# karpathy/minbpe

Measured on NVIDIA H100. Metric: train_loop_corpus_GBps, higher is better.
Workload: dtype int32

## Files before the change

### minbpe_b200/csrc/b200bpe.cu

```cuda
#include <algorithm>
#include <cstdio>
#include <cstdlib>
#include <cstring>
#include <new>
#include <string>
#include <vector>

#include "../../include/b200bpe.h"
#include "common.cuh"
#include "k_load.cuh"
#include "k_merge.cuh"
#include "k_merge_seg.cuh"
#include "k_seg.cuh"
#include "k_seg_filter.cuh"
#include "k_stats.cuh"
#include "k_encode.cuh"
#include "k_split.cuh"
#include "k_decode.cuh"
#include "k_xchg.cuh"
#include "k_encode2.cuh"
#include "k_special.cuh"
#include "k_weighted.cuh"
#include "k_dedup.cuh"

#define BPE_ABI_VERSION 4

struct EncState;
struct SpecSet;
struct GenEnc;
struct DdSession;
struct bpe_handle {
    int device = 0;
    EncState *enc = nullptr;
    bpe_handle *enc_scratch = nullptr;
    SpecSet *spec = nullptr;
    GenEnc *gen = nullptr;
    DdSession *dd = nullptr;
    int sms = 0;
    cudaStream_t stream = nullptr;
    cudaStream_t own_stream = nullptr;
    std::string err;

    u32 *buf[2] = {nullptr, nullptr};
    u64 cap_tokens = 0;
    bool loaded = false;
    bool bytes_only = false;
    bool weighted = false;
    u64 *wts = nullptr; u64 wts_cap = 0, n_entries = 0;
    u32 *wt_cnt = nullptr; u64 *wt_base = nullptr; u64 wt_seg_cap = 0;
    bool wt_fresh = false;

    Ctl *ctl = nullptr;
    Ctl *h_ctl = nullptr;

    Table table = {nullptr, nullptr, nullptr, 0};
    bool table_valid = false;
    u64 *desc = nullptr; u64 desc_cap = 0;
    Edge *edge[2] = {nullptr, nullptr}; u64 *seg_offs = nullptr; u64 seg_cap = 0;
    ull *delta = nullptr; u32 V = 0;
    u32 delta_cap = 0;
    u32 delta_vecs = 0;
    bool batching = false;
    u32 max_id = 255;
    ull *dense = nullptr;
    ull *dense2 = nullptr; u32 *d_cmp = nullptr;
    int hist_mode = 0;
    u32 *sig = nullptr, *cand = nullptr; u64 sig_cap = 0;
    bool filt_active = false;
    bool sig_valid = false;
    u32 *d_err = nullptr;
    int *log_pairs = nullptr; long long *log_counts = nullptr; int log_cap = 0;
    Best *partials = nullptr;
    TopList *top_partials = nullptr;
    unsigned char *d_cls = nullptr, *d_contr = nullptr;
    unsigned char *xchg = nullptr; u64 xchg_bytes = 0, xchg_stride = 0; u32 xchg_V = 0;
    XArgs xargs = {};
    bool xchg_attached = false;
    u32 *d_present = nullptr;
    unsigned char *split_slab = nullptr; u64 split_cap = 0;
    int argmax_grid = 0, merge_grid_same = 0, merge_grid_seg = 0, ff_grid = 0;

    int step_poll_every = 16;
    int opt_kernel_timing = 0, opt_rescan = 0, opt_batch = 256, opt_table_log2 = 0;
    int opt_memo_log2 = 0;
    u32 opt_vocab_cap = 0;
    int opt_seg_filter = 0;
    int opt_hist_kernel = 2;
    int opt_dedup_log2 = 0;
    u64 dd_stats[8] = {};
    int opt_split_pattern = 0;

    bpe_timing tm = {};
    std::vector<cudaEvent_t> ev_pool;
    int ev_used = 0;
};

static thread_local std::string g_create_err;
static void xchg_release(bpe_handle *h);
static void enc2_free(bpe_handle *h);
static void spec_free(bpe_handle *h);
static void gen_free(bpe_handle *h);
static void dd_free(bpe_handle *h);
static u64 g_split_piece_override = 0;

static int fail(bpe_handle *h, int code, const std::string &msg) {
    if (h) h->err = msg; else g_create_err = msg;
    return code;
}

#define CU(call)                                                                                   \
    do {                                                                                           \
        cudaError_t e_ = (call);                                                                   \
        if (e_ != cudaSuccess)                                                                     \
            return fail(h, BPE_ERR_CUDA, std::string(#call) + ": " + cudaGetErrorString(e_));      \
    } while (0)

static inline int grid_for(u64 work_items, int threads, int max_blocks) {
    u64 b = (work_items + threads - 1) / threads;
    if (b < 1) b = 1;
    if (b > (u64)max_blocks) b = max_blocks;
    return (int)b;
}

extern "C" int bpe_abi_version(void) { return BPE_ABI_VERSION; }

extern "C" const char *bpe_last_error(const bpe_handle *h) { return h ? h->err.c_str() : g_create_err.c_str(); }

static int free_table(bpe_handle *h, Table &t) {
    if (t.keys) cudaFree(t.keys);
    if (t.counts) cudaFree(t.counts);
    if (t.first) cudaFree(t.first);
    t = {nullptr, nullptr, nullptr, 0};
    (void)h;
    return BPE_OK;
}

static int alloc_table(bpe_handle *h, Table &t, u64 cap, bool with_first) {
    t = {nullptr, nullptr, nullptr, cap - 1};
    CU(cudaMalloc(&t.keys, cap * 8));
    CU(cudaMalloc(&t.counts, cap * 8));
    if (with_first) CU(cudaMalloc(&t.first, cap * 8));
    CU(cudaMemsetAsync(t.keys, 0xff, cap * 8, h->stream));
    CU(cudaMemsetAsync(t.counts, 0, cap * 8, h->stream));
    if (with_first) CU(cudaMemsetAsync(t.first, 0xff, cap * 8, h->stream));
    return BPE_OK;
}

static u64 next_pow2(u64 x) { u64 p = 1; while (p < x) p <<= 1; return p; }

extern "C" int bpe_create(int device, bpe_handle **out) {
    bpe_handle *h = nullptr;
    if (!out) return fail(nullptr, BPE_ERR_ARG, "bpe_create: out is NULL");
    *out = nullptr;
    int ndev = 0;
    cudaError_t e = cudaGetDeviceCount(&ndev);
    if (e != cudaSuccess || ndev == 0)
        return fail(nullptr, BPE_ERR_CUDA, std::string("bpe_create: no CUDA device (") + cudaGetErrorString(e) +
                                               "); libb200bpe has no CPU fallback");
    if (device < 0 || device >= ndev) return fail(nullptr, BPE_ERR_ARG, "bpe_create: device index out of range");
    cudaDeviceProp prop;
    e = cudaGetDeviceProperties(&prop, device);
    if (e != cudaSuccess) return fail(nullptr, BPE_ERR_CUDA, cudaGetErrorString(e));
    if (prop.major != 9 || prop.minor != 0)
        return fail(nullptr, BPE_ERR_CUDA, std::string("bpe_create: device '") + prop.name + "' is sm_" +
                                               std::to_string(prop.major) + std::to_string(prop.minor) +
                                               "; this library contains sm_90a code only");
    h = new (std::nothrow) bpe_handle();
    if (!h) return fail(nullptr, BPE_ERR_INTERNAL, "out of host memory");
    h->device = device;
    h->sms = prop.multiProcessorCount;
    auto bail = [&](const char *what, cudaError_t ce) {
        std::string m = std::string(what) + ": " + cudaGetErrorString(ce);
        delete h;
        return fail(nullptr, BPE_ERR_CUDA, m);
    };
    if ((e = cudaSetDevice(device)) != cudaSuccess) return bail("cudaSetDevice", e);
    if ((e = cudaStreamCreateWithFlags(&h->own_stream, cudaStreamNonBlocking)) != cudaSuccess) return bail("cudaStreamCreate", e);
    h->stream = h->own_stream;
    if ((e = cudaMalloc(&h->ctl, sizeof(Ctl))) != cudaSuccess) return bail("cudaMalloc ctl", e);
    if ((e = cudaMallocHost(&h->h_ctl, sizeof(Ctl))) != cudaSuccess) return bail("cudaMallocHost", e);
    if ((e = cudaMalloc(&h->dense, 65536 * 8)) != cudaSuccess) return bail("cudaMalloc dense", e);
    if ((e = cudaMalloc(&h->d_err, 8)) != cudaSuccess) return bail("cudaMalloc err", e);
    int occ_same = 1;
    cudaOccupancyMaxActiveBlocksPerMultiprocessor(&occ_same, k_merge<true>, MG_THREADS, 0);
    if (occ_same < 1) occ_same = 1;
    h->merge_grid_same = h->sms * occ_same;
    int occ_fast = 0;
    if ((e = cudaFuncSetAttribute(k_merge_seg<false>, cudaFuncAttributeMaxDynamicSharedMemorySize, MS_SMEM_BYTES)) != cudaSuccess)
        return bail("cudaFuncSetAttribute(k_merge_seg)", e);
    cudaOccupancyMaxActiveBlocksPerMultiprocessor(&occ_fast, k_merge_seg<false>, MS_THREADS, MS_SMEM_BYTES);
    if (occ_fast < 1) return bail("k_merge_seg does not fit on an SM", cudaErrorLaunchOutOfResources);
    h->merge_grid_seg = h->sms * occ_fast;
    h->argmax_grid = h->sms * 2;
    h->ff_grid = h->sms * 4;
    if ((e = cudaMalloc(&h->partials, sizeof(Best) * h->argmax_grid)) != cudaSuccess) return bail("cudaMalloc partials", e);
    if ((e = cudaMalloc(&h->top_partials, sizeof(TopList) * h->argmax_grid)) != cudaSuccess) return bail("cudaMalloc top_partials", e);
    memset(h->h_ctl, 0, sizeof(Ctl));
    h->h_ctl->epoch = 1;
    h->h_ctl->found_pos = POS_NONE;
    if ((e = cudaMemcpy(h->ctl, h->h_ctl, sizeof(Ctl), cudaMemcpyHostToDevice)) != cudaSuccess) return bail("cudaMemcpy ctl", e);
    *out = h;
    return BPE_OK;
}

extern "C" int bpe_destroy(bpe_handle *h) {
    if (!h) return BPE_OK;
    cudaSetDevice(h->device);
    cudaStreamSynchronize(h->stream);
    for (int i = 0; i < 2; ++i) if (h->buf[i]) cudaFree(h->buf[i]);
    for (cudaEvent_t e : h->ev_pool) cudaEventDestroy(e);
    free_table(h, h->table);
    if (h->desc) cudaFree(h->desc);
    for (int i = 0; i < 2; ++i) if (h->edge[i]) cudaFree(h->edge[i]);
    if (h->seg_offs) cudaFree(h->seg_offs);
    if (h->sig) cudaFree(h->sig);
    if (h->cand) cudaFree(h->cand);
    if (h->delta) cudaFree(h->delta);
    if (h->dense) cudaFree(h->dense);
    if (h->dense2) cudaFree(h->dense2);
    if (h->d_cmp) cudaFree(h->d_cmp);
    if (h->d_err) cudaFree(h->d_err);
    if (h->log_pairs) cudaFree(h->log_pairs);
    if (h->log_counts) cudaFree(h->log_counts);
    if (h->partials) cudaFree(h->partials);
    if (h->top_partials) cudaFree(h->top_partials);
    if (h->d_cls) cudaFree(h->d_cls);
    if (h->d_contr) cudaFree(h->d_contr);
    if (h->d_present) cudaFree(h->d_present);
    if (h->wts) cudaFree(h->wts);
    if (h->wt_cnt) cudaFree(h->wt_cnt);
    if (h->wt_base) cudaFree(h->wt_base);
    xchg_release(h);
    enc2_free(h);
    spec_free(h);
    gen_free(h);
    dd_free(h);
    if (h->enc_scratch) bpe_destroy(h->enc_scratch);
    if (h->split_slab) cudaFree(h->split_slab);
    if (h->ctl) cudaFree(h->ctl);
    if (h->h_ctl) cudaFreeHost(h->h_ctl);
    if (h->own_stream) cudaStreamDestroy(h->own_stream);
    delete h;
    return BPE_OK;
}

extern "C" int bpe_set_option(bpe_handle *h, int opt, int64_t value) {
    if (!h) return BPE_ERR_ARG;
    switch (opt) {
        case BPE_OPT_KERNEL_TIMING: h->opt_kernel_timing = value != 0; break;
        case BPE_OPT_RESCAN: h->opt_rescan = value != 0; break;
        case BPE_OPT_BATCH: h->opt_batch = (int)std::max<int64_t>(1, std::min<int64_t>(value, 4096)); break;
        case BPE_OPT_TABLE_LOG2:
            if (value != 0 && (value < 10 || value > 30)) return fail(h, BPE_ERR_ARG, "table log2 must be 0 or in [10,30]");
            h->opt_table_log2 = (int)value; break;
        case BPE_OPT_VOCAB_CAP:
            if (value < 0 || value >= 0x3fffffff) return fail(h, BPE_ERR_ARG, "vocabulary capacity out of range");
            h->opt_vocab_cap = (u32)value; break;
        case BPE_OPT_ENC_MEMO_LOG2:
            if (value != 0 && (value < 6 || value > 28)) return fail(h, BPE_ERR_ARG, "memo log2 must be 0 or in [6,28]");
            h->opt_memo_log2 = (int)value;
            cudaSetDevice(h->device); cudaStreamSynchronize(h->stream);
            enc2_free(h);
            break;
        case BPE_OPT_SEG_FILTER:
            if (value < 0 || value > 2) return fail(h, BPE_ERR_ARG, "segment filter must be 0 (off), 1 (when sparse) or 2 (always)");
            h->opt_seg_filter = (int)value; h->filt_active = false; h->sig_valid = false;
            break;
        case BPE_OPT_HIST_KERNEL:
            if (value < 0 || value > 2) return fail(h, BPE_ERR_ARG, "hist kernel must be 0 (auto), 1 (packed) or 2 (hashed)");
            h->opt_hist_kernel = (int)value;
            if (value == 0) h->hist_mode = 0;
            break;
        case BPE_OPT_SPLIT_PATTERN:
            if (value != 0 && value != 1) return fail(h, BPE_ERR_ARG, "split pattern must be 0 (GPT-4) or 1 (GPT-2)");
            h->opt_split_pattern = (int)value; break;
        case BPE_OPT_DEDUP_LOG2:
            if (value != 0 && (value < 4 || value > 30)) return fail(h, BPE_ERR_ARG, "dedup log2 must be 0 or in [4,30]");
            h->opt_dedup_log2 = (int)value; break;
        case BPE_OPT_SPLIT_PIECE:
            if (value != 0 && value < 4096) return fail(h, BPE_ERR_ARG, "split piece must be 0 (default) or >= 4096 bytes");
            g_split_piece_override = (u64)value; break;
        default: return fail(h, BPE_ERR_ARG, "unknown option");
    }
    return BPE_OK;
}

extern "C" int bpe_get_timing(bpe_handle *h, bpe_timing *out) {
    if (!h || !out) return BPE_ERR_ARG;
    *out = h->tm;
    return BPE_OK;
}

static int ensure_stream_capacity(bpe_handle *h, u64 n) {
    const u64 need = ((n + MG_TILE - 1) / MG_TILE + 1) * MG_TILE;
    if (need > h->cap_tokens) {
        if (h->split_slab) { cudaFree(h->split_slab); h->split_slab = nullptr; h->split_cap = 0; }
        for (int i = 0; i < 2; ++i) { if (h->buf[i]) cudaFree(h->buf[i]); h->buf[i] = nullptr; }
        h->cap_tokens = 0;
        for (int i = 0; i < 2; ++i) CU(cudaMalloc(&h->buf[i], need * 4));
        h->cap_tokens = need;
    }
    const u64 tiles = need / MG_TILE + 1;
    if (tiles > h->desc_cap) {
        if (h->desc) cudaFree(h->desc);
        h->desc = nullptr; h->desc_cap = 0;
        CU(cudaMalloc(&h->desc, tiles * 8));
        CU(cudaMemsetAsync(h->desc, 0, tiles * 8, h->stream));
        h->desc_cap = tiles;
    }
    const u64 segs = need / SEG_TOKENS + 1;
    if (segs > h->seg_cap) {
        for (int i = 0; i < 2; ++i) { if (h->edge[i]) cudaFree(h->edge[i]); h->edge[i] = nullptr; }
        if (h->seg_offs) cudaFree(h->seg_offs);
        h->seg_offs = nullptr; h->seg_cap = 0;
        for (int i = 0; i < 2; ++i) CU(cudaMalloc(&h->edge[i], segs * sizeof(Edge)));
        CU(cudaMalloc(&h->seg_offs, segs * 8));
        h->seg_cap = segs;
    }
    return BPE_OK;
}

static int build_edges(bpe_handle *h, u64 n) {
    const u64 nseg = (n + SEG_TOKENS - 1) / SEG_TOKENS;
    k_build_edges<<<grid_for(nseg, 256, h->sms * 4), 256, 0, h->stream>>>(h->buf[0], h->buf[1], h->ctl, h->edge[0], 0);
    CU(cudaGetLastError());
    return BPE_OK;
}

static void enqueue_pack(bpe_handle *h, int force) {
    k_scan_counts<<<1, 1024, 0, h->stream>>>(h->ctl, h->edge[0], h->edge[1], h->seg_offs, force);
    k_gather<<<h->sms * 8, 256, 0, h->stream>>>(h->ctl, h->buf[0], h->buf[1], h->edge[0], h->edge[1], h->seg_offs, nullptr, force, 1);
    h->tm.kernel_launches += 2;
}
static void enqueue_edges_after_contig(bpe_handle *h) {
    k_build_edges<<<h->sms * 4, 256, 0, h->stream>>>(h->buf[0], h->buf[1], h->ctl, h->edge[0], 1);
    h->tm.kernel_launches += 1;
}

static void enqueue_wt_bases(bpe_handle *h, int force) {
    k_wt_marks<<<h->sms * 8, 256, 0, h->stream>>>(h->buf[0], h->buf[1], h->ctl, h->edge[0], h->edge[1], h->wt_cnt, force);
    k_wt_scan<<<1, 1024, 0, h->stream>>>(h->ctl, h->wt_cnt, h->wt_base, force);
    h->tm.kernel_launches += 2;
}

static int push_ctl(bpe_handle *h) {
    CU(cudaMemcpyAsync(h->ctl, h->h_ctl, sizeof(Ctl), cudaMemcpyHostToDevice, h->stream));
    return BPE_OK;
}
static int pull_ctl(bpe_handle *h) {
    CU(cudaMemcpyAsync(h->h_ctl, h->ctl, sizeof(Ctl), cudaMemcpyDeviceToHost, h->stream));
    CU(cudaStreamSynchronize(h->stream));
    return BPE_OK;
}

static int reset_ctl_for_stream(bpe_handle *h, u64 n) {
    int rc = pull_ctl(h);
    if (rc) return rc;
    const u32 epoch = h->h_ctl->epoch ? h->h_ctl->epoch : 1;
    memset(h->h_ctl, 0, sizeof(Ctl));
    h->h_ctl->epoch = epoch;
    h->h_ctl->n = n;
    h->h_ctl->found_pos = POS_NONE;
    h->h_ctl->first_idx = 256;
    return push_ctl(h);
}

static int check_offsets(bpe_handle *h, const uint64_t *offs, uint64_t k, uint64_t n) {
    if (!offs || k == 0) return BPE_OK;
    if (offs[0] != 0) return fail(h, BPE_ERR_ARG, "chunk_offsets[0] must be 0");
    for (u64 i = 1; i < k; ++i)
        if (offs[i] <= offs[i - 1] || offs[i] >= n) return fail(h, BPE_ERR_ARG, "chunk_offsets must be strictly increasing and < n");
    return BPE_OK;
}

static int mark_chunks(bpe_handle *h, u32 *dst, const uint64_t *offs, uint64_t k, uint64_t n) {
    u64 zero = 0;
    if (!offs || k == 0) { offs = &zero; k = n ? 1 : 0; }
    if (k == 0) return BPE_OK;
    const u64 piece = 1ull << 24;
    u64 *d_offs = nullptr;
    CU(cudaMalloc(&d_offs, std::min(piece, k) * 8));
    for (u64 s = 0; s < k; s += piece) {
        const u64 m = std::min(piece, k - s);
        cudaError_t e = cudaMemcpyAsync(d_offs, offs + s, m * 8, cudaMemcpyHostToDevice, h->stream);
        if (e == cudaSuccess) {
            k_set_flags<<<grid_for(m, 256, h->sms * 8), 256, 0, h->stream>>>(dst, d_offs, m, n);
            e = cudaStreamSynchronize(h->stream);
        }
        if (e != cudaSuccess) { cudaFree(d_offs); return fail(h, BPE_ERR_CUDA, std::string("mark_chunks: ") + cudaGetErrorString(e)); }
        h->tm.h2d_bytes += m * 8;
    }
    cudaFree(d_offs);
    return BPE_OK;
}

static int load_bytes_into(bpe_handle *h, u32 *dst, const uint8_t *bytes, uint64_t n, const unsigned char *d_perm) {
    const u64 piece = 1ull << 28;
    unsigned char *d_bytes = nullptr;
    if (n == 0) return BPE_OK;
    CU(cudaMalloc(&d_bytes, std::min(piece, n)));
    for (u64 s = 0; s < n; s += piece) {
        const u64 m = std::min(piece, n - s);
        cudaError_t e = cudaMemcpyAsync(d_bytes, bytes + s, m, cudaMemcpyHostToDevice, h->stream);
        if (e == cudaSuccess) {
            k_widen_bytes<<<grid_for(m / 16 + 1, 256, h->sms * 8), 256, 0, h->stream>>>(d_bytes, dst + s, m, d_perm);
            e = cudaStreamSynchronize(h->stream);
        }
        if (e != cudaSuccess) { cudaFree(d_bytes); return fail(h, BPE_ERR_CUDA, std::string("load_bytes: ") + cudaGetErrorString(e)); }
        h->tm.h2d_bytes += m;
    }
    cudaFree(d_bytes);
    return BPE_OK;
}

extern "C" int bpe_load_stream(bpe_handle *h, const uint8_t *bytes, uint64_t n, const uint64_t *chunk_offsets,
                               uint64_t n_chunks) {
    if (!h) return BPE_ERR_ARG;
    if (!bytes && n) return fail(h, BPE_ERR_ARG, "bytes is NULL");
    if (n >= (1ull << 36)) return fail(h, BPE_ERR_ARG, "stream too long (limit 2^36 tokens)");
    CU(cudaSetDevice(h->device));
    int rc = check_offsets(h, chunk_offsets, n_chunks, n);
    if (rc) return rc;
    h->tm.h2d_bytes = 0;
    h->loaded = false; h->table_valid = false; h->weighted = false;
    if ((rc = ensure_stream_capacity(h, n))) return rc;
    if ((rc = load_bytes_into(h, h->buf[0], bytes, n, nullptr))) return rc;
    if ((rc = mark_chunks(h, h->buf[0], chunk_offsets, n_chunks, n))) return rc;
    if ((rc = reset_ctl_for_stream(h, n))) return rc;
    if ((rc = build_edges(h, n))) return rc;
    h->loaded = true; h->bytes_only = true; h->max_id = 255;
    return BPE_OK;
}

extern "C" int bpe_load_ids(bpe_handle *h, const int32_t *ids, uint64_t n, const uint64_t *chunk_offsets,
                            uint64_t n_chunks) {
    if (!h) return BPE_ERR_ARG;
    if (!ids && n) return fail(h, BPE_ERR_ARG, "ids is NULL");
    if (n >= (1ull << 36)) return fail(h, BPE_ERR_ARG, "stream too long (limit 2^36 tokens)");
    CU(cudaSetDevice(h->device));
    int rc = check_offsets(h, chunk_offsets, n_chunks, n);
    if (rc) return rc;
    h->tm.h2d_bytes = 0;
    h->loaded = false; h->table_valid = false; h->weighted = false;
    if ((rc = ensure_stream_capacity(h, n))) return rc;
    h->max_id = 0;
    if (n) {
        CU(cudaMemcpyAsync(h->buf[1], ids, n * 4, cudaMemcpyHostToDevice, h->stream));
        CU(cudaMemsetAsync(h->d_err, 0, 8, h->stream));
        k_copy_ids<<<grid_for(n, 256, h->sms * 8), 256, 0, h->stream>>>((const int *)h->buf[1], h->buf[0], n, h->d_err);
        u32 bad[2] = {0, 0};
        CU(cudaMemcpyAsync(bad, h->d_err, 8, cudaMemcpyDeviceToHost, h->stream));
        CU(cudaStreamSynchronize(h->stream));
        if (bad[0]) return fail(h, BPE_ERR_ARG, "ids must be in [0, 2^31-1)");
        h->max_id = bad[1];
        h->tm.h2d_bytes += n * 4;
    }
    if ((rc = mark_chunks(h, h->buf[0], chunk_offsets, n_chunks, n))) return rc;
    if ((rc = reset_ctl_for_stream(h, n))) return rc;
    if ((rc = build_edges(h, n))) return rc;
    h->loaded = true; h->bytes_only = false;
    return BPE_OK;
}

extern "C" int bpe_stream_len(bpe_handle *h, uint64_t *n) {
    if (!h || !n) return BPE_ERR_ARG;
    if (!h->loaded) return fail(h, BPE_ERR_STATE, "no stream loaded");
    CU(cudaSetDevice(h->device));
    int rc = pull_ctl(h);
    if (rc) return rc;
    *n = h->h_ctl->n;
    return BPE_OK;
}

extern "C" int bpe_read_stream(bpe_handle *h, int32_t *out, uint64_t cap, uint64_t *n) {
    if (!h || !n) return BPE_ERR_ARG;
    if (!h->loaded) return fail(h, BPE_ERR_STATE, "no stream loaded");
    CU(cudaSetDevice(h->device));
    int rc = pull_ctl(h);
    if (rc) return rc;
    const u64 len = h->h_ctl->n;
    *n = len;
    if (cap < len) return fail(h, BPE_ERR_CAPACITY, "output buffer too small");
    if (len == 0) return BPE_OK;
    if (!out) return fail(h, BPE_ERR_ARG, "out is NULL");
    const u32 cur = h->h_ctl->cur;
    k_scan_counts<<<1, 1024, 0, h->stream>>>(h->ctl, h->edge[0], h->edge[1], h->seg_offs, 1);
    k_gather<<<h->sms * 8, 256, 0, h->stream>>>(h->ctl, h->buf[0], h->buf[1], h->edge[0], h->edge[1], h->seg_offs,
                                                 h->buf[cur ^ 1], 1, 0);
    k_strip_flags<<<grid_for(len, 256, h->sms * 8), 256, 0, h->stream>>>(h->buf[cur ^ 1], (int *)h->buf[cur ^ 1], len);
    CU(cudaMemcpyAsync(out, h->buf[cur ^ 1], len * 4, cudaMemcpyDeviceToHost, h->stream));
    CU(cudaStreamSynchronize(h->stream));
// ... 530 lines not shown
```

### minbpe_b200/csrc/k_merge_seg.cuh

```cuda
#pragma once
#include "common.cuh"
#include "k_merge.cuh"
#include "k_seg.cuh"

#ifndef MS_WARPS
#define MS_WARPS 8
#endif
#define MS_THREADS (MS_WARPS * 32)
#ifndef MS_STAGES
#define MS_STAGES 2
#endif
#ifndef MS_MINBLOCKS
#define MS_MINBLOCKS 4
#endif
#ifndef MS_DCACHE_LOG2
#define MS_DCACHE_LOG2 9
#endif
#ifndef MS_BATCH
#define MS_BATCH 8
#endif
#define MS_PAD 4
#define MS_SW (SEG_TOKENS + 8)
#define MS_META 16
#define MS_BE (MS_BATCH + 2)
#define MS_DCACHE (1 << MS_DCACHE_LOG2)
#define MS_WARP_WORDS (MS_STAGES * MS_SW + MS_STAGES * MS_META + MS_BE * 8)
#define MS_SMEM_BYTES (MS_WARPS * MS_WARP_WORDS * 4 + MS_WARPS * MS_STAGES * 8 + MS_DCACHE * 8 + 16 + BATCH_MAX * 8)
#define MS_INVALID 0xffffffffu
static_assert(SEG_TOKENS == 512, "k_merge_seg: a lane owns 4 rows x 4 tokens of a 512-token segment");
static_assert((MS_SW * 4) % 16 == 0 && (MS_WARP_WORDS * 4) % 16 == 0, "bulk-copy destinations must stay 16-byte aligned");

__device__ __noinline__ void delta_cache_add(u32 *s_dkey, u32 *s_dcnt, ull *delta, u32 idx) {
    u32 slot = (idx * 2654435761u) >> (32 - MS_DCACHE_LOG2);
#pragma unroll 1
    for (int probe = 0; probe < 4; ++probe) {
        u32 k = reinterpret_cast<volatile u32 *>(s_dkey)[slot];
        if (k == 0xffffffffu) {
            const u32 old = atomicCAS(&s_dkey[slot], 0xffffffffu, idx);
            k = (old == 0xffffffffu) ? idx : old;
        }
        if (k == idx) { atomicAdd(&s_dcnt[slot], 1u); return; }
        slot = (slot + 1) & (MS_DCACHE - 1);
    }
    atomicAdd(&delta[idx], 1ull);
}

__device__ __noinline__ void delta_one(u32 at, u32 a, u32 b, u32 V, u32 *s_dkey, u32 *s_dcnt, ull *delta) {
    const u32 t0 = lds32(at), tm1 = lds32o<-4>(at), tm2 = lds32o<-8>(at), tp2 = lds32o<8>(at), tp3 = lds32o<12>(at);
    const bool m_m2 = (((tm2 ^ a) & TOK_MASK) == 0) && tm1 == b;
    const bool m_p2 = (((tp2 ^ a) & TOK_MASK) == 0) && tp3 == b;
    if (tm1 != TOK_SENTINEL && !(t0 & TOK_FLAG) && !m_m2) delta_cache_add(s_dkey, s_dcnt, delta, tm1 & TOK_MASK);
    if (!(tp2 & TOK_FLAG))
        delta_cache_add(s_dkey, s_dcnt, delta, m_p2 ? 2u * V : V + tp2);
}

__device__ __forceinline__ u32 batch_member(u32 tok, u32 nk, u32 mem_a) {
    u32 j = 0;
#pragma unroll 1
    for (; j < nk; ++j) if (lds32(mem_a + 8 * j) == (tok & TOK_MASK)) break;
    return j;
}
__device__ __forceinline__ u32 batch_start(u32 t, u32 nx, u32 nk, u32 mem_a) {
    const u32 j = batch_member(t, nk, mem_a);
    return (j < nk && lds32(mem_a + 8 * j + 4) == nx) ? j : nk;
}

__device__ __noinline__ void delta_batch(u32 at, u32 nk, u32 mem_a, u32 z, u32 V, u32 *s_dkey, u32 *s_dcnt, ull *delta) {
    const u32 t0 = lds32(at), tm1 = lds32o<-4>(at), tm2 = lds32o<-8>(at), tp2 = lds32o<8>(at), tp3 = lds32o<12>(at);
    const u32 j = batch_member(t0, nk, mem_a);
    const u32 ml = batch_start(tm2, tm1, nk, mem_a);
    const u32 mr = batch_start(tp2, tp3, nk, mem_a);
    const u32 base = j * (2u * V + 1u);
    if (tm1 != TOK_SENTINEL && !(t0 & TOK_FLAG) && ml != j)
        delta_cache_add(s_dkey, s_dcnt, delta, base + (ml < j ? z + ml : tm1 & TOK_MASK));
    if (!(tp2 & TOK_FLAG))
        delta_cache_add(s_dkey, s_dcnt, delta, base + (mr == j ? 2u * V : V + (mr < j ? z + mr : tp2)));
}

struct SegArgs {
    Ctl *ctl;
    u32 *buf0, *buf1;
    Edge *e0, *e1;
    ull *delta;
    u32 V;
    int force;
    int batched;
    const unsigned char *xbase;
    u64 xstride;
};

template <int R, bool BATCH>
__device__ __forceinline__ void mark_row(u32 la, u32 lane, u32 count, u32 a, u32 b, u32 z, u32 nk, u32 mem_a, u32 (&t)[4],
                                         u32 &mn, u32 &keep, u32 &dirty) {
    const uint4 q = lds128o<R * 512>(la);
    const u32 nx = lds32o<R * 512 + 16>(la), pv = lds32o<R * 512 - 4>(la);
    t[0] = q.x; t[1] = q.y; t[2] = q.z; t[3] = q.w;
    u32 m = 0, pm = 0;
#pragma unroll 1
    for (u32 j = 0; j < (BATCH ? nk : 1u); ++j) {
        if (BATCH) { a = lds32(mem_a + 8 * j); b = lds32(mem_a + 8 * j + 4); }
        m |= (((t[0] ^ a) & TOK_MASK) == 0 && t[1] == b) ? 1u : 0u;
        m |= (((t[1] ^ a) & TOK_MASK) == 0 && t[2] == b) ? 2u : 0u;
        m |= (((t[2] ^ a) & TOK_MASK) == 0 && t[3] == b) ? 4u : 0u;
        m |= (((t[3] ^ a) & TOK_MASK) == 0 && nx == b) ? 8u : 0u;
        pm |= (((pv ^ a) & TOK_MASK) == 0 && t[0] == b) ? 1u : 0u;
    }
    const u32 d = ((m << 1) | pm) & 0xfu;
    u32 valid = 0xfu;
    if (R * 128u + 128u > count) {
        const int rem = (int)count - (int)(R * 128 + lane * 4);
        valid = rem >= 4 ? 0xfu : (rem <= 0 ? 0u : ((1u << rem) - 1u));
    }
    mn = m & valid;
    keep = ~d & valid;
    dirty |= (mn | (keep ^ valid)) ? (1u << R) : 0u;
    if (mn) {
        auto zof = [&](u32 x) { return (BATCH ? z + batch_member(x, nk, mem_a) : z) | (x & TOK_FLAG); };
        if (mn & 1u) t[0] = zof(t[0]);
        if (mn & 2u) t[1] = zof(t[1]);
        if (mn & 4u) t[2] = zof(t[2]);
        if (mn & 8u) t[3] = zof(t[3]);
    }
}

__device__ __forceinline__ void scatter_row(u32 s_a, u32 lane, u32 off, u32 row_kept, u32 lane_excl, u32 kp, const u32 (&t)[4]) {
    if (row_kept == 128u) {
        const u32 p = s_a + ((off + 4u * lane) << 2);
        if ((off & 3u) == 0) sts128(p, t[0], t[1], t[2], t[3]);
        else { sts32(p, t[0]); sts32o<4>(p, t[1]); sts32o<8>(p, t[2]); sts32o<12>(p, t[3]); }
    } else {
        u32 p = s_a + ((off + lane_excl) << 2);
        if (kp & 1u) sts32(p, t[0]);
        p += (kp << 2) & 4u;
        if (kp & 2u) sts32(p, t[1]);
        p += (kp << 1) & 4u;
        if (kp & 4u) sts32(p, t[2]);
        p += kp & 4u;
        if (kp & 8u) sts32(p, t[3]);
    }
}

template <bool LIST>
__global__ void __launch_bounds__(MS_THREADS, MS_MINBLOCKS) k_merge_seg(SegArgs A) {
    Ctl *ctl = A.ctl;
    if (!A.force && (ctl->done || ctl->overflow || ctl->iter >= ctl->max_iter)) return;
    if (ctl->a == ctl->b) return;

    extern __shared__ __align__(128) unsigned char smem_raw[];
    u32 *s_warp = reinterpret_cast<u32 *>(smem_raw);
    u64 *s_bar = reinterpret_cast<u64 *>(s_warp + MS_WARPS * MS_WARP_WORDS);
    u32 *s_dkey = reinterpret_cast<u32 *>(s_bar + MS_WARPS * MS_STAGES);
    u32 *s_dcnt = s_dkey + MS_DCACHE;
    ull *s_drops = reinterpret_cast<ull *>(s_dcnt + MS_DCACHE);
    u32 *s_mem = reinterpret_cast<u32 *>(s_drops + 1);

    const u32 FULL = 0xffffffffu;
    const u32 tid = threadIdx.x, lane = tid & 31, warp = tid >> 5;
    const u64 n = ctl->n;
    u32 *__restrict__ w = ctl->cur ? A.buf1 : A.buf0;
    const Edge *__restrict__ e_cur = ctl->edge_cur ? A.e1 : A.e0;
    Edge *__restrict__ e_next = ctl->edge_cur ? A.e0 : A.e1;
    const u32 a = (u32)ctl->a, b = (u32)ctl->b, z = (u32)ctl->z;
    const u32 nseg = ctl->nseg;
    const u32 nk = (!LIST && A.batched) ? ctl->nk : 1u;
    const u32 mem_a = smem_addr(s_mem);
    ull *const delta = A.xbase ? x_local_delta(A.xbase, A.xstride) : A.delta;
    const u32 *__restrict__ cand = LIST ? reinterpret_cast<const u32 *>(ctl->cand_ptr) : nullptr;
    const u32 n_cand = LIST ? ctl->n_cand : 0u;

    const u32 ws_a = smem_addr(s_warp + warp * MS_WARP_WORDS);
    const u32 wmeta_a = ws_a + MS_STAGES * MS_SW * 4;
    const u32 wbe_a = wmeta_a + MS_STAGES * MS_META * 4;
    const u32 wbar_a = smem_addr(s_bar + warp * MS_STAGES);

    if (lane == 0) {
        for (int s = 0; s < MS_STAGES; ++s) mbar_init(s_bar + warp * MS_STAGES + s, 1);
        fence_mbar_init();
    }
    for (u32 i = tid; i < MS_DCACHE; i += MS_THREADS) { s_dkey[i] = 0xffffffffu; s_dcnt[i] = 0; }
    if (tid == 0) *s_drops = 0;
    if (tid < nk) { s_mem[2 * tid] = tid ? (u32)ctl->bat_a[tid] : a; s_mem[2 * tid + 1] = tid ? (u32)ctl->bat_b[tid] : b; }
    __syncthreads();

    u32 batch_seg = 0, batch_pos = MS_BATCH;
    u32 list_next = blockIdx.x * MS_WARPS + warp;
    const u32 meta_src = 4u * (lane == 0 ? 4u : lane == 1 ? 3u : lane < 5 ? 14u + lane : lane < 8 ? 0u : lane < 16 ? lane : 0u);
    bool exhausted = false;
    auto issue = [&](u32 stage) {
        const u32 meta_a = wmeta_a + stage * (MS_META * 4);
        for (;;) {
            if (exhausted) {
                if (lane == 0) sts32o<20>(meta_a, MS_INVALID);
                __syncwarp();
                return;
            }
            if (batch_pos == MS_BATCH) {
                u32 tk = 0;
                if (LIST) {
                    tk = list_next; list_next += gridDim.x * MS_WARPS;
                    if (tk >= n_cand) { exhausted = true; continue; }
                    batch_seg = cand[tk] - (MS_BATCH - 1); batch_pos = MS_BATCH - 1;
                } else {
                    if (lane == 0) tk = atomicAdd(&ctl->merge_ticket, 1u);
                    tk = __shfl_sync(FULL, tk, 0);
                    if ((u64)tk * MS_BATCH >= nseg) { exhausted = true; continue; }
                    batch_seg = tk * MS_BATCH; batch_pos = 0;
                }
                if (LIST ? (lane >= MS_BATCH - 1 && lane < MS_BE) : (lane < MS_BE)) {
                    const long long idx = (LIST ? (long long)(int)batch_seg : (long long)batch_seg) - 1 + lane;
                    uint4 q0, q1;
                    if (idx >= 0 && idx < (long long)nseg) {
                        const uint4 *p = reinterpret_cast<const uint4 *>(&e_cur[idx]);
                        q0 = p[0]; q1 = p[1];
                    } else {
                        q0 = make_uint4(TOK_SENTINEL, TOK_SENTINEL, TOK_SENTINEL, TOK_SENTINEL);
                        q1 = make_uint4(TOK_SENTINEL, 3u, 0u, 0u);
                    }
                    sts128(wbe_a + lane * 32, q0.x, q0.y, q0.z, q0.w);
                    sts128(wbe_a + lane * 32 + 16, q1.x, q1.y, q1.z, q1.w);
                }
                __syncwarp();
            }
            const u32 k = batch_pos++;
            const u32 seg = batch_seg + k;
            if (seg >= nseg) { exhausted = true; continue; }
            const u32 rec_a = wbe_a + k * 32;
            const u32 cnt = lds32o<32 + 20>(rec_a);
            if (cnt == 0) {
                if (lane < 8) reinterpret_cast<u32 *>(&e_next[seg])[lane] = (lane < 5) ? TOK_SENTINEL : 0u;
                continue;
            }
            const u32 cm1 = lds32o<20>(rec_a), cp1 = lds32o<64 + 20>(rec_a);
            const u32 st_a = ws_a + stage * (MS_SW * 4);
            u32 mv = lds32(rec_a + meta_src);
            if (lane == 5) mv = seg;
            if (lane == 6) mv = cnt;
            if (lane < 16) sts32(meta_a + lane * 4, mv);
            if (lane < 2) sts32(st_a + (MS_PAD - 1 - lane) * 4, mv);
            if (!(cm1 >= 2 && cp1 >= 3)) {
                __syncwarp();
                if (lane == 0) {
                    u32 N[3], P[2];
                    seg_neighbours(e_cur, seg, nseg, N, P);
                    sts32o<0>(meta_a, P[0]); sts32o<4>(meta_a, P[1]); sts32o<8>(meta_a, N[0]); sts32o<12>(meta_a, N[1]); sts32o<16>(meta_a, N[2]);
                    sts32o<(MS_PAD - 1) * 4>(st_a, P[0]); sts32o<(MS_PAD - 2) * 4>(st_a, P[1]);
                }
            }
            __syncwarp();
            if (lane == 0) {
                const u32 bytes = ((cnt + 3u) & ~3u) * 4u;
                fence_proxy_async_smem();
                mbar_arrive_expect_tx_a(wbar_a + stage * 8, bytes);
                bulk_g2s_a(st_a + MS_PAD * 4, w + (u64)seg * SEG_TOKENS, bytes, wbar_a + stage * 8);
            }
            __syncwarp();
            return;
        }
    };

    for (u32 s = 0; s + 1 < MS_STAGES; ++s) issue(s);
    u32 drops = 0;
    for (u32 j = 0;; ++j) {
        const u32 stage = j % MS_STAGES;
        issue((j + MS_STAGES - 1) % MS_STAGES);
        const u32 meta_a = wmeta_a + stage * (MS_META * 4);
        const u32 seg = lds32o<20>(meta_a);
        if (seg == MS_INVALID) break;
        const u32 count = lds32o<24>(meta_a);
        const u32 s_a = ws_a + stage * (MS_SW * 4) + MS_PAD * 4;
        mbar_wait_a(wbar_a + stage * 8, (j / MS_STAGES) & 1u);
        if (lane < 3) sts32(s_a + (count + lane) * 4, lds32(meta_a + 8 + lane * 4));
        __syncwarp();

        u32 t[4][4], mn[4] = {0, 0, 0, 0}, keep[4] = {0, 0, 0, 0};
        u32 dirty = 0;
        const u32 la = s_a + lane * 16;
        if (nk == 1u) {
            mark_row<0, false>(la, lane, count, a, b, z, 1u, mem_a, t[0], mn[0], keep[0], dirty);
            if (count > 128u) mark_row<1, false>(la, lane, count, a, b, z, 1u, mem_a, t[1], mn[1], keep[1], dirty);
            if (count > 256u) mark_row<2, false>(la, lane, count, a, b, z, 1u, mem_a, t[2], mn[2], keep[2], dirty);
            if (count > 384u) mark_row<3, false>(la, lane, count, a, b, z, 1u, mem_a, t[3], mn[3], keep[3], dirty);
        } else {
            mark_row<0, true>(la, lane, count, a, b, z, nk, mem_a, t[0], mn[0], keep[0], dirty);
            if (count > 128u) mark_row<1, true>(la, lane, count, a, b, z, nk, mem_a, t[1], mn[1], keep[1], dirty);
            if (count > 256u) mark_row<2, true>(la, lane, count, a, b, z, nk, mem_a, t[2], mn[2], keep[2], dirty);
            if (count > 384u) mark_row<3, true>(la, lane, count, a, b, z, nk, mem_a, t[3], mn[3], keep[3], dirty);
        }
        dirty = __reduce_or_sync(FULL, dirty);
        if (!dirty) {
            if (lane < 8) reinterpret_cast<u32 *>(&e_next[seg])[lane] = lds32(meta_a + 32 + lane * 4);
            __syncwarp();
            continue;
        }

        if (delta) {
            u32 mall = mn[0] | (mn[1] << 4) | (mn[2] << 8) | (mn[3] << 12);
#pragma unroll 1
            while (mall) {
                const int bit = __ffs(mall) - 1;
                mall &= mall - 1;
                const u32 at = la + (bit >> 2) * 512 + (bit & 3) * 4;
                if (nk == 1u) delta_one(at, a, b, A.V, s_dkey, s_dcnt, delta);
                else delta_batch(at, nk, mem_a, z, A.V, s_dkey, s_dcnt, delta);
            }
        }

        const u32 own = __popc(keep[0]) | (__popc(keep[1]) << 8) | (__popc(keep[2]) << 16) | (__popc(keep[3]) << 24);
        u32 incl = own;
#pragma unroll
        for (int o = 1; o < 32; o <<= 1) {
            const u32 v = __shfl_up_sync(FULL, incl, o);
            if (lane >= (u32)o) incl += v;
        }
        const u32 tot = __shfl_sync(FULL, incl, 31);
        const u32 excl = incl - own;
        const u32 k0 = tot & 0xffu, k1 = (tot >> 8) & 0xffu, k2 = (tot >> 16) & 0xffu, k3 = tot >> 24;
        const u32 off1 = k0, off2 = k0 + k1, off3 = off2 + k2;
        const u32 new_count = off3 + k3;
        const int first_dirty = __ffs(dirty) - 1;
        __syncwarp();

        if (first_dirty <= 0) scatter_row(s_a, lane, 0u, k0, excl & 0xffu, keep[0], t[0]);
        if (first_dirty <= 1 && count > 128u) scatter_row(s_a, lane, off1, k1, (excl >> 8) & 0xffu, keep[1], t[1]);
        if (first_dirty <= 2 && count > 256u) scatter_row(s_a, lane, off2, k2, (excl >> 16) & 0xffu, keep[2], t[2]);
        if (count > 384u) scatter_row(s_a, lane, off3, k3, excl >> 24, keep[3], t[3]);
        __syncwarp();
        {
            uint4 *__restrict__ gp = reinterpret_cast<uint4 *>(w + (u64)seg * SEG_TOKENS) + lane;
            const u32 vend = (new_count + 3u) >> 2;
            if (first_dirty <= 0 && lane < vend) gp[0] = lds128o<0>(la);
            if (first_dirty <= 1 && lane + 32u < vend) gp[32] = lds128o<512>(la);
            if (first_dirty <= 2 && lane + 64u < vend) gp[64] = lds128o<1024>(la);
            if (lane + 96u < vend) gp[96] = lds128o<1536>(la);
        }
        {
            const u32 idx = lane < 3 ? lane : new_count + lane - 5u;
            const bool have = lane < 3 ? (lane < new_count) : (new_count + lane >= 5u);
            u32 word = TOK_SENTINEL;
            if (have && lane < 5) word = lds32(s_a + (idx & (SEG_TOKENS - 1)) * 4);
            if (lane == 5) word = new_count;
            if (lane > 5) word = 0;
            if (lane < 8) reinterpret_cast<u32 *>(&e_next[seg])[lane] = word;
        }
        drops += count - new_count;
        __syncwarp();
    }

    if (lane == 0 && drops) atomicAdd(s_drops, (ull)drops);
    __syncthreads();
    if (delta)
        for (u32 i = tid; i < MS_DCACHE; i += MS_THREADS)
            if (s_dkey[i] != 0xffffffffu && s_dcnt[i]) atomicAdd(&delta[s_dkey[i]], (ull)s_dcnt[i]);
    if (tid == 0) {
        const ull cta_drops = *s_drops;
        if (cta_drops) atomicAdd(&ctl->drops, cta_drops);
        __threadfence();
        const u32 e = atomicAdd(&ctl->merge_exit, 1u);
        if (e == gridDim.x - 1) {
            __threadfence();
            const ull dropped = *(volatile ull *)&ctl->drops;
            ctl->sum_in += n; ctl->sum_out += n - dropped;
            ctl->n = n - dropped;
            ctl->drops = 0;
            ctl->edge_cur ^= 1u;
            ctl->iter += nk;
            ctl->epoch += 1;
            ctl->merge_ticket = 0; ctl->merge_exit = 0;
        }
    }
}
```

Before: 637.7.

## Specialize merge kernel per batch size and warp-parallelize delta updates

```diff
diff --git a/minbpe_b200/csrc/b200bpe.cu b/minbpe_b200/csrc/b200bpe.cu
--- a/minbpe_b200/csrc/b200bpe.cu
+++ b/minbpe_b200/csrc/b200bpe.cu
@@ -186,7 +186,8 @@
     if (occ_same < 1) occ_same = 1;
     h->merge_grid_same = h->sms * occ_same;
     int occ_fast = 0;
-    if ((e = cudaFuncSetAttribute(k_merge_seg<false>, cudaFuncAttributeMaxDynamicSharedMemorySize, MS_SMEM_BYTES)) != cudaSuccess)
+    if ((e = cudaFuncSetAttribute(k_merge_seg<false>, cudaFuncAttributeMaxDynamicSharedMemorySize, MS_SMEM_BYTES)) != cudaSuccess ||
+        (e = cudaFuncSetAttribute(k_merge_seg<true>, cudaFuncAttributeMaxDynamicSharedMemorySize, MS_SMEM_BYTES)) != cudaSuccess)
         return bail("cudaFuncSetAttribute(k_merge_seg)", e);
     cudaOccupancyMaxActiveBlocksPerMultiprocessor(&occ_fast, k_merge_seg<false>, MS_THREADS, MS_SMEM_BYTES);
     if (occ_fast < 1) return bail("k_merge_seg does not fit on an SM", cudaErrorLaunchOutOfResources);
diff --git a/minbpe_b200/csrc/k_merge_seg.cuh b/minbpe_b200/csrc/k_merge_seg.cuh
--- a/minbpe_b200/csrc/k_merge_seg.cuh
+++ b/minbpe_b200/csrc/k_merge_seg.cuh
@@ -24,13 +24,14 @@
 #define MS_META 16
 #define MS_BE (MS_BATCH + 2)
 #define MS_DCACHE (1 << MS_DCACHE_LOG2)
-#define MS_WARP_WORDS (MS_STAGES * MS_SW + MS_STAGES * MS_META + MS_BE * 8)
-#define MS_SMEM_BYTES (MS_WARPS * MS_WARP_WORDS * 4 + MS_WARPS * MS_STAGES * 8 + MS_DCACHE * 8 + 16 + BATCH_MAX * 8)
+#define MS_LIST (SEG_TOKENS / 2)
+#define MS_WARP_WORDS (MS_STAGES * MS_SW + MS_STAGES * MS_META + MS_BE * 8 + MS_LIST)
+#define MS_SMEM_BYTES (MS_WARPS * MS_WARP_WORDS * 4 + MS_WARPS * MS_STAGES * 8 + MS_DCACHE * 8 + 16)
 #define MS_INVALID 0xffffffffu
 static_assert(SEG_TOKENS == 512, "k_merge_seg: a lane owns 4 rows x 4 tokens of a 512-token segment");
 static_assert((MS_SW * 4) % 16 == 0 && (MS_WARP_WORDS * 4) % 16 == 0, "bulk-copy destinations must stay 16-byte aligned");
 
-__device__ __noinline__ void delta_cache_add(u32 *s_dkey, u32 *s_dcnt, ull *delta, u32 idx) {
+__device__ __noinline__ void delta_cache_add(u32 *s_dkey, u32 *s_dcnt, ull *delta, u32 idx, u32 cnt) {
     u32 slot = (idx * 2654435761u) >> (32 - MS_DCACHE_LOG2);
 #pragma unroll 1
     for (int probe = 0; probe < 4; ++probe) {
@@ -39,42 +40,91 @@
             const u32 old = atomicCAS(&s_dkey[slot], 0xffffffffu, idx);
             k = (old == 0xffffffffu) ? idx : old;
         }
-        if (k == idx) { atomicAdd(&s_dcnt[slot], 1u); return; }
+        if (k == idx) { atomicAdd(&s_dcnt[slot], cnt); return; }
         slot = (slot + 1) & (MS_DCACHE - 1);
     }
-    atomicAdd(&delta[idx], 1ull);
-}
-
-__device__ __noinline__ void delta_one(u32 at, u32 a, u32 b, u32 V, u32 *s_dkey, u32 *s_dcnt, ull *delta) {
+    atomicAdd(&delta[idx], (ull)cnt);
+}
+
+template <int NK>
+struct Members {
+    u32 a[NK], b[NK];
+};
+
+template <int NK>
+__device__ __forceinline__ u32 member_of(const Members<NK> &M, u32 x, u32 &bj) {
+    u32 j = NK;
+    bj = 0;
+#pragma unroll
+    for (int k = 0; k < NK; ++k)
+        if ((x & TOK_MASK) == M.a[k]) { j = k; bj = M.b[k]; }
+    return j;
+}
+template <int NK>
+__device__ __forceinline__ bool starts(const Members<NK> &M, u32 x, u32 y) {
+    if constexpr (NK == 1) {
+        return ((x ^ M.a[0]) & TOK_MASK) == 0 && y == M.b[0];
+    } else {
+        x &= TOK_MASK;
+        u32 r = TOK_MASK;
+#pragma unroll
+        for (int k = 0; k < NK; ++k) r = x == M.a[k] ? M.b[k] : r;
+        return y == r;
+    }
+}
+template <int NK>
+__device__ __forceinline__ u32 start_of(const Members<NK> &M, u32 x, u32 y) {
+    u32 bj;
+    const u32 j = member_of(M, x, bj);
+    return (j < NK && y == bj) ? j : NK;
+}
+
+template <int NK>
+__device__ __forceinline__ void start_delta(u32 at, const Members<NK> &M, u32 z, u32 V, u32 &li, u32 &ri) {
     const u32 t0 = lds32(at), tm1 = lds32o<-4>(at), tm2 = lds32o<-8>(at), tp2 = lds32o<8>(at), tp3 = lds32o<12>(at);
-    const bool m_m2 = (((tm2 ^ a) & TOK_MASK) == 0) && tm1 == b;
-    const bool m_p2 = (((tp2 ^ a) & TOK_MASK) == 0) && tp3 == b;
-    if (tm1 != TOK_SENTINEL && !(t0 & TOK_FLAG) && !m_m2) delta_cache_add(s_dkey, s_dcnt, delta, tm1 & TOK_MASK);
-    if (!(tp2 & TOK_FLAG))
-        delta_cache_add(s_dkey, s_dcnt, delta, m_p2 ? 2u * V : V + tp2);
-}
-
-__device__ __forceinline__ u32 batch_member(u32 tok, u32 nk, u32 mem_a) {
-    u32 j = 0;
+    u32 bj;
+    const u32 j = NK == 1 ? 0u : member_of(M, t0, bj);
+    const u32 ml = start_of(M, tm2, tm1);
+    const u32 mr = start_of(M, tp2, tp3);
+    const u32 base = j * (2u * V + 1u);
+    li = (tm1 != TOK_SENTINEL && !(t0 & TOK_FLAG) && ml != j) ? base + (ml < j ? z + ml : tm1 & TOK_MASK) : MS_INVALID;
+    ri = !(tp2 & TOK_FLAG)
+             ? base + (mr == j ? 2u * V : V + (mr < j ? z + mr : tp2)) : MS_INVALID;
+}
+
+__device__ __forceinline__ void delta_fold_add(u32 idx, u32 lane, u32 *s_dkey, u32 *s_dcnt, ull *delta) {
+    const u32 grp = __match_any_sync(0xffffffffu, idx);
+    if (idx != MS_INVALID && lane == (u32)(__ffs(grp) - 1)) delta_cache_add(s_dkey, s_dcnt, delta, idx, (u32)__popc(grp));
+}
+
+template <int NK>
+__device__ __forceinline__ void segment_delta(u32 s_a, u32 list_a, u32 lane, u32 mall, const Members<NK> &M, u32 z, u32 V,
+                                              u32 *s_dkey, u32 *s_dcnt, ull *delta) {
+    const u32 own = __popc(mall);
+    u32 incl = own;
+#pragma unroll
+    for (int o = 1; o < 32; o <<= 1) {
+        const u32 v = __shfl_up_sync(0xffffffffu, incl, o);
+        if (lane >= (u32)o) incl += v;
+    }
+    const u32 total = __shfl_sync(0xffffffffu, incl, 31);
+    u32 p = list_a + (incl - own) * 4u;
 #pragma unroll 1
-    for (; j < nk; ++j) if (lds32(mem_a + 8 * j) == (tok & TOK_MASK)) break;
-    return j;
-}
-__device__ __forceinline__ u32 batch_start(u32 t, u32 nx, u32 nk, u32 mem_a) {
-    const u32 j = batch_member(t, nk, mem_a);
-    return (j < nk && lds32(mem_a + 8 * j + 4) == nx) ? j : nk;
-}
-
-__device__ __noinline__ void delta_batch(u32 at, u32 nk, u32 mem_a, u32 z, u32 V, u32 *s_dkey, u32 *s_dcnt, ull *delta) {
-    const u32 t0 = lds32(at), tm1 = lds32o<-4>(at), tm2 = lds32o<-8>(at), tp2 = lds32o<8>(at), tp3 = lds32o<12>(at);
-    const u32 j = batch_member(t0, nk, mem_a);
-    const u32 ml = batch_start(tm2, tm1, nk, mem_a);
-    const u32 mr = batch_start(tp2, tp3, nk, mem_a);
-    const u32 base = j * (2u * V + 1u);
-    if (tm1 != TOK_SENTINEL && !(t0 & TOK_FLAG) && ml != j)
-        delta_cache_add(s_dkey, s_dcnt, delta, base + (ml < j ? z + ml : tm1 & TOK_MASK));
-    if (!(tp2 & TOK_FLAG))
-        delta_cache_add(s_dkey, s_dcnt, delta, base + (mr == j ? 2u * V : V + (mr < j ? z + mr : tp2)));
+    while (mall) {
+        const u32 bit = __ffs(mall) - 1;
+        mall &= mall - 1;
+        sts32(p, (bit >> 2) * 512u + lane * 16u + (bit & 3u) * 4u);
+        p += 4u;
+    }
+    __syncwarp();
+#pragma unroll 1
+    for (u32 base = 0; base < total; base += 32u) {
+        u32 li = MS_INVALID, ri = MS_INVALID;
+        if (base + lane < total) start_delta(s_a + lds32(list_a + (base + lane) * 4u), M, z, V, li, ri);
+        delta_fold_add(li, lane, s_dkey, s_dcnt, delta);
+        delta_fold_add(ri, lane, s_dkey, s_dcnt, delta);
+    }
+    __syncwarp();
 }
 
 struct SegArgs {
@@ -89,22 +139,16 @@
     u64 xstride;
 };
 
-template <int R, bool BATCH>
-__device__ __forceinline__ void mark_row(u32 la, u32 lane, u32 count, u32 a, u32 b, u32 z, u32 nk, u32 mem_a, u32 (&t)[4],
-                                         u32 &mn, u32 &keep, u32 &dirty) {
+template <int R, int NK>
+__device__ __forceinline__ void mark_row(u32 la, u32 lane, u32 count, const Members<NK> &M, u32 z, u32 (&t)[4],
+                                         u32 &mn, u32 &keep, u32 &dirty, u32 &up) {
     const uint4 q = lds128o<R * 512>(la);
-    const u32 nx = lds32o<R * 512 + 16>(la), pv = lds32o<R * 512 - 4>(la);
+    const u32 nx = lds32o<R * 512 + 16>(la);
     t[0] = q.x; t[1] = q.y; t[2] = q.z; t[3] = q.w;
-    u32 m = 0, pm = 0;
-#pragma unroll 1
-    for (u32 j = 0; j < (BATCH ? nk : 1u); ++j) {
-        if (BATCH) { a = lds32(mem_a + 8 * j); b = lds32(mem_a + 8 * j + 4); }
-        m |= (((t[0] ^ a) & TOK_MASK) == 0 && t[1] == b) ? 1u : 0u;
-        m |= (((t[1] ^ a) & TOK_MASK) == 0 && t[2] == b) ? 2u : 0u;
-        m |= (((t[2] ^ a) & TOK_MASK) == 0 && t[3] == b) ? 4u : 0u;
-        m |= (((t[3] ^ a) & TOK_MASK) == 0 && nx == b) ? 8u : 0u;
-        pm |= (((pv ^ a) & TOK_MASK) == 0 && t[0] == b) ? 1u : 0u;
-    }
+    const u32 m = (starts(M, t[0], t[1]) ? 1u : 0u) | (starts(M, t[1], t[2]) ? 2u : 0u) | (starts(M, t[2], t[3]) ? 4u : 0u) |
+                  (starts(M, t[3], nx) ? 8u : 0u);
+    const u32 pm = __shfl_sync(0xffffffffu, lane == 31 ? up : m, (lane + 31) & 31) >> 3;
+    up = m;
     const u32 d = ((m << 1) | pm) & 0xfu;
     u32 valid = 0xfu;
     if (R * 128u + 128u > count) {
@@ -115,7 +159,12 @@
     keep = ~d & valid;
     dirty |= (mn | (keep ^ valid)) ? (1u << R) : 0u;
     if (mn) {
-        auto zof = [&](u32 x) { return (BATCH ? z + batch_member(x, nk, mem_a) : z) | (x & TOK_FLAG); };
+        auto zof = [&](u32 x) {
+            u32 id = z;
+#pragma unroll
+            for (int j = 1; j < NK; ++j) if ((x & TOK_MASK) == M.a[j]) id = z + j;
+            return id | (x & TOK_FLAG);
+        };
         if (mn & 1u) t[0] = zof(t[0]);
         if (mn & 2u) t[1] = zof(t[1]);
         if (mn & 4u) t[2] = zof(t[2]);
@@ -140,19 +189,15 @@
     }
 }
 
-template <bool LIST>
-__global__ void __launch_bounds__(MS_THREADS, MS_MINBLOCKS) k_merge_seg(SegArgs A) {
+template <bool LIST, int NK>
+__device__ __forceinline__ void merge_seg_pass(const SegArgs &A) {
     Ctl *ctl = A.ctl;
-    if (!A.force && (ctl->done || ctl->overflow || ctl->iter >= ctl->max_iter)) return;
-    if (ctl->a == ctl->b) return;
-
     extern __shared__ __align__(128) unsigned char smem_raw[];
     u32 *s_warp = reinterpret_cast<u32 *>(smem_raw);
     u64 *s_bar = reinterpret_cast<u64 *>(s_warp + MS_WARPS * MS_WARP_WORDS);
     u32 *s_dkey = reinterpret_cast<u32 *>(s_bar + MS_WARPS * MS_STAGES);
     u32 *s_dcnt = s_dkey + MS_DCACHE;
     ull *s_drops = reinterpret_cast<ull *>(s_dcnt + MS_DCACHE);
-    u32 *s_mem = reinterpret_cast<u32 *>(s_drops + 1);
 
     const u32 FULL = 0xffffffffu;
     const u32 tid = threadIdx.x, lane = tid & 31, warp = tid >> 5;
@@ -160,10 +205,14 @@
     u32 *__restrict__ w = ctl->cur ? A.buf1 : A.buf0;
     const Edge *__restrict__ e_cur = ctl->edge_cur ? A.e1 : A.e0;
     Edge *__restrict__ e_next = ctl->edge_cur ? A.e0 : A.e1;
-    const u32 a = (u32)ctl->a, b = (u32)ctl->b, z = (u32)ctl->z;
+    const u32 z = (u32)ctl->z;
     const u32 nseg = ctl->nseg;
-    const u32 nk = (!LIST && A.batched) ? ctl->nk : 1u;
-    const u32 mem_a = smem_addr(s_mem);
+    Members<NK> M;
+#pragma unroll
+    for (int j = 0; j < NK; ++j) {
+        M.a[j] = j ? (u32)ctl->bat_a[j] : (u32)ctl->a;
+        M.b[j] = j ? (u32)ctl->bat_b[j] : (u32)ctl->b;
+    }
     ull *const delta = A.xbase ? x_local_delta(A.xbase, A.xstride) : A.delta;
     const u32 *__restrict__ cand = LIST ? reinterpret_cast<const u32 *>(ctl->cand_ptr) : nullptr;
     const u32 n_cand = LIST ? ctl->n_cand : 0u;
@@ -171,6 +220,7 @@
     const u32 ws_a = smem_addr(s_warp + warp * MS_WARP_WORDS);
     const u32 wmeta_a = ws_a + MS_STAGES * MS_SW * 4;
     const u32 wbe_a = wmeta_a + MS_STAGES * MS_META * 4;
+    const u32 wlist_a = wbe_a + MS_BE * 32;
     const u32 wbar_a = smem_addr(s_bar + warp * MS_STAGES);
 
     if (lane == 0) {
@@ -179,7 +229,6 @@
     }
     for (u32 i = tid; i < MS_DCACHE; i += MS_THREADS) { s_dkey[i] = 0xffffffffu; s_dcnt[i] = 0; }
     if (tid == 0) *s_drops = 0;
-    if (tid < nk) { s_mem[2 * tid] = tid ? (u32)ctl->bat_a[tid] : a; s_mem[2 * tid + 1] = tid ? (u32)ctl->bat_b[tid] : b; }
     __syncthreads();
 
     u32 batch_seg = 0, batch_pos = MS_BATCH;
@@ -275,17 +324,11 @@
         u32 t[4][4], mn[4] = {0, 0, 0, 0}, keep[4] = {0, 0, 0, 0};
         u32 dirty = 0;
         const u32 la = s_a + lane * 16;
-        if (nk == 1u) {
-            mark_row<0, false>(la, lane, count, a, b, z, 1u, mem_a, t[0], mn[0], keep[0], dirty);
-            if (count > 128u) mark_row<1, false>(la, lane, count, a, b, z, 1u, mem_a, t[1], mn[1], keep[1], dirty);
-            if (count > 256u) mark_row<2, false>(la, lane, count, a, b, z, 1u, mem_a, t[2], mn[2], keep[2], dirty);
-            if (count > 384u) mark_row<3, false>(la, lane, count, a, b, z, 1u, mem_a, t[3], mn[3], keep[3], dirty);
-        } else {
-            mark_row<0, true>(la, lane, count, a, b, z, nk, mem_a, t[0], mn[0], keep[0], dirty);
-            if (count > 128u) mark_row<1, true>(la, lane, count, a, b, z, nk, mem_a, t[1], mn[1], keep[1], dirty);
-            if (count > 256u) mark_row<2, true>(la, lane, count, a, b, z, nk, mem_a, t[2], mn[2], keep[2], dirty);
-            if (count > 384u) mark_row<3, true>(la, lane, count, a, b, z, nk, mem_a, t[3], mn[3], keep[3], dirty);
-        }
+        u32 up = starts(M, lds32o<-4>(s_a), lds32(s_a)) ? 8u : 0u;
+        mark_row<0>(la, lane, count, M, z, t[0], mn[0], keep[0], dirty, up);
+        if (count > 128u) mark_row<1>(la, lane, count, M, z, t[1], mn[1], keep[1], dirty, up);
+        if (count > 256u) mark_row<2>(la, lane, count, M, z, t[2], mn[2], keep[2], dirty, up);
+        if (count > 384u) mark_row<3>(la, lane, count, M, z, t[3], mn[3], keep[3], dirty, up);
         dirty = __reduce_or_sync(FULL, dirty);
         if (!dirty) {
             if (lane < 8) reinterpret_cast<u32 *>(&e_next[seg])[lane] = lds32(meta_a + 32 + lane * 4);
@@ -293,17 +336,8 @@
             continue;
         }
 
-        if (delta) {
-            u32 mall = mn[0] | (mn[1] << 4) | (mn[2] << 8) | (mn[3] << 12);
-#pragma unroll 1
-            while (mall) {
-                const int bit = __ffs(mall) - 1;
-                mall &= mall - 1;
-                const u32 at = la + (bit >> 2) * 512 + (bit & 3) * 4;
-                if (nk == 1u) delta_one(at, a, b, A.V, s_dkey, s_dcnt, delta);
-                else delta_batch(at, nk, mem_a, z, A.V, s_dkey, s_dcnt, delta);
-            }
-        }
+        if (delta)
+            segment_delta(s_a, wlist_a, lane, mn[0] | (mn[1] << 4) | (mn[2] << 8) | (mn[3] << 12), M, z, A.V, s_dkey, s_dcnt, delta);
 
         const u32 own = __popc(keep[0]) | (__popc(keep[1]) << 8) | (__popc(keep[2]) << 16) | (__popc(keep[3]) << 24);
         u32 incl = own;
@@ -363,9 +397,27 @@
             ctl->n = n - dropped;
             ctl->drops = 0;
             ctl->edge_cur ^= 1u;
-            ctl->iter += nk;
+            ctl->iter += NK;
             ctl->epoch += 1;
             ctl->merge_ticket = 0; ctl->merge_exit = 0;
         }
     }
 }
+
+template <bool LIST>
+__global__ void __launch_bounds__(MS_THREADS, MS_MINBLOCKS) k_merge_seg(SegArgs A) {
+    const Ctl *ctl = A.ctl;
+    if (!A.force && (ctl->done || ctl->overflow || ctl->iter >= ctl->max_iter)) return;
+    if (ctl->a == ctl->b) return;
+    static_assert(BATCH_MAX == 4, "k_merge_seg: one pass per member count 1..BATCH_MAX");
+    if constexpr (LIST) {
+        merge_seg_pass<true, 1>(A);
+    } else {
+        switch (A.batched ? ctl->nk : 1u) {
+        case 2: merge_seg_pass<false, 2>(A); break;
+        case 3: merge_seg_pass<false, 3>(A); break;
+        case 4: merge_seg_pass<false, 4>(A); break;
+        default: merge_seg_pass<false, 1>(A); break;
+        }
+    }
+}
```

Result: faster. 743.2 (median of 6 runs) (+16.5%).
